# robflynnyh/long-context-asr

Hardware: AMD Instinct MI355X
Metric: spectrogram-frames/sec (6L/768D, seq=16384) (higher is better)
Workload: dtype bf16; 1 GPU; 6L/768D/6H SConformerXL, seq=16384, rotary theta=1.5M, fwd+CTC+bwd+clip+MADGRAD; per_gpu_batch=128, global_batch=128, seq_len=16384, parallelism=dp1

## Files before the change

long-context-asr_amd/csrc/gemm256.hip:

```cpp
#ifdef SCONF_GEMM_STAMP
#define SCONF_STAMPS
#endif
#include "gemm_tile.h"
#include <algorithm>
#include <stdio.h>

namespace {
using namespace gemm_tile;

constexpr int TM = 256, TK = 64;
constexpr int HT = 128 * 64 * 2;
constexpr int BUF = 4 * HT;
constexpr int GM2 = 4;

__device__ __forceinline__ int swz_a(int row) { return (row >> 1) & 7; }
__device__ __forceinline__ int swz_b(int row) { return ((row >> 1) & 1) | (((row >> 3) & 3) << 1); }
__device__ __forceinline__ int swz_b1n(int row) { return ((row >> 1) & 1) | (((row >> 2) & 3) << 1); }

template <bool KS, bool BOP, int JH> struct DmaOffs {
    unsigned off[2][2];
    __device__ __forceinline__ void set(long ld, int tid, bool rot = false) {
        constexpr int WC = 32 + 16 * JH;
#pragma unroll
        for (int h = 0; h < 2; ++h)
#pragma unroll
            for (int i = 0; i < 2; ++i) {
                const int c = tid + 512 * i;
                if (!KS) {
                    const int row = c >> 3, pos = c & 7;
                    int kc, mrow;
                    if (!BOP)              { kc = pos ^ swz_a(row); mrow = 128 * h + row; }
                    else if (h == 0)       { kc = pos ^ swz_b(row); mrow = rot ? 128 * (row >> 6) + 32 * ((row >> 5) & 1) + (row & 31) : WC * (row >> 5) + (row & 31); }
                    else if (JH == 2)      { kc = pos ^ swz_b(row); mrow = rot ? 128 * (row >> 6) + 32 * ((row >> 5) & 1) + 64 + (row & 31) : WC * (row >> 5) + 32 + (row & 31); }
                    else                   { kc = pos ^ swz_b1n(row & 63); mrow = WC * ((row & 63) >> 4) + 32 + (row & 15); }
                    off[h][i] = (unsigned)(((long)mrow * ld + kc * 8) * 2);
                } else {
                    const int kr = c >> 4, pos = c & 15, rc = pos ^ swz_strided(kr);
                    off[h][i] = (unsigned)(((long)kr * ld + 128 * h + rc * 8) * 2);
                }
            }
    }
};
template <int NP>
__device__ __forceinline__ void dma_half(const char* base, const unsigned (&off)[2], char* dst, int tid) {
#pragma unroll
    for (int i = 0; i < NP; ++i)
        __builtin_amdgcn_global_load_lds((gptr)(base + off[i]), (lptr)(dst + ((tid & ~63) + 512 * i) * 16), 16, 0, 0);
}

__device__ __forceinline__ bf16x4 lds_read_tr(const char* p) {
    bf16x4 v;
    asm volatile("ds_read_b64_tr_b16 %0, %1" : "=v"(v) : "v"(lds_addr(p)));
    return v;
}
template <int OFF> __device__ __forceinline__ bf16x4 lds_read_tr_off(unsigned a) {
    bf16x4 v;
    asm volatile("ds_read_b64_tr_b16 %0, %1 offset:%2" : "=v"(v) : "v"(a), "n"(OFF));
    return v;
}
__device__ __forceinline__ void frag_pair_ks(const char* s, int col, int lane, bf16x8& f0, bf16x8& f1) {
    const int a = lane & 15, q = a >> 2, g = lane >> 4;
    const int chunk = col >> 3, sub = (col & 4) * 2, k0 = 8 * g + q;
    const unsigned base = lds_addr(s + k0 * 256 + ((chunk ^ swz_strided(k0)) << 4) + sub);
    const bf16x4 l0 = lds_read_tr_off<0>(base), h0 = lds_read_tr_off<1024>(base);
    const bf16x4 l1 = lds_read_tr_off<8192>(base), h1 = lds_read_tr_off<9216>(base);
    f0 = __builtin_shufflevector(l0, h0, 0, 1, 2, 3, 4, 5, 6, 7);
    f1 = __builtin_shufflevector(l1, h1, 0, 1, 2, 3, 4, 5, 6, 7);
}
template <bool KS> __device__ __forceinline__ bf16x8 frag_a(const char* s, int wr, int i, int kk, int lane) {
    if (!KS) {
        const int r = 64 * wr + 16 * i + (lane & 15), c = kk * 4 + (lane >> 4);
        return *reinterpret_cast<const bf16x8*>(s + r * 128 + ((c ^ swz_a(r)) << 4));
    } else {
        const int a = lane & 15, q = a >> 2, pp = a & 3, g = lane >> 4;
        const int col = 64 * wr + 16 * i + 4 * pp, chunk = col >> 3, sub = (col & 4) * 2;
        const int k0 = kk * 32 + 8 * g + q, k1 = k0 + 4;
        bf16x4 lo = lds_read_tr(s + k0 * 256 + ((chunk ^ swz_strided(k0)) << 4) + sub);
        bf16x4 hi = lds_read_tr(s + k1 * 256 + ((chunk ^ swz_strided(k1)) << 4) + sub);
        return __builtin_shufflevector(lo, hi, 0, 1, 2, 3, 4, 5, 6, 7);
    }
}
template <bool KS, bool NARROW> __device__ __forceinline__ bf16x8 frag_b(const char* s, int wc, int j, int kk, int lane) {
    if (!KS) {
        const int a = lane & 15, c = kk * 4 + (lane >> 4);
        if (!NARROW) {
            const int r = 32 * wc + 8 * (a >> 2) + 4 * j + (a & 3);
            return *reinterpret_cast<const bf16x8*>(s + r * 128 + ((c ^ swz_b(r)) << 4));
        } else {
            const int r = 16 * wc + 4 * (a >> 2) + (a & 3);
            return *reinterpret_cast<const bf16x8*>(s + r * 128 + ((c ^ swz_b1n(r)) << 4));
        }
    } else {
        const int a = lane & 15, q = a >> 2, pp = a & 3, g = lane >> 4;
        const int col = 32 * wc + 16 * j + 4 * pp, chunk = col >> 3, sub = (col & 4) * 2;
        const int k0 = kk * 32 + 8 * g + q, k1 = k0 + 4;
        bf16x4 lo = lds_read_tr(s + k0 * 256 + ((chunk ^ swz_strided(k0)) << 4) + sub);
        bf16x4 hi = lds_read_tr(s + k1 * 256 + ((chunk ^ swz_strided(k1)) << 4) + sub);
        return __builtin_shufflevector(lo, hi, 0, 1, 2, 3, 4, 5, 6, 7);
    }
}

struct Item { int m0, n0, kbeg, nkt, split; };
struct Sched { int total, ntiles, tiles_m, tiles_n, tn, gm; };
__device__ __forceinline__ Item item_coords(const GemmParams& p, const Sched& sc, int v) {
    const int qx = sc.total >> 3, rx = sc.total & 7, xcd = v & 7;
    const int lid = (xcd < rx ? xcd * (qx + 1) : rx * (qx + 1) + (xcd - rx) * qx) + (v >> 3);
    const int split = lid / sc.ntiles, t = lid - split * sc.ntiles;
    const int per_group = sc.gm * sc.tiles_n;
    const int g = t / per_group, r = t - g * per_group;
    const int first_m = g * sc.gm, gm = min(sc.gm, sc.tiles_m - first_m);
    Item w;
    w.m0 = (first_m + r % gm) * TM; w.n0 = (r / gm) * sc.tn;
    w.split = split;
    w.kbeg = split * p.k_per_split;
    w.nkt = (min(p.K, w.kbeg + p.k_per_split) - w.kbeg) / TK;
    return w;
}
struct Cursor {
    int v, kt, par; bool valid; Item it;
    __device__ __forceinline__ void advance(const GemmParams& p, const Sched& sc) {
        par ^= 1;
        if (++kt < it.nkt) return;
        kt = 0; v += gridDim.x;
        if (v < sc.total) it = item_coords(p, sc, v); else valid = false;
    }
};

template <int W> struct RawBf;
template <> struct RawBf<8> { typedef bf16x8 type; };
template <> struct RawBf<4> { typedef bf16x4 type; };
template <int ACT, bool RES, bool KS, int JH, int FL = -1, bool ROT = false, int DEEP = 0>
__device__ __forceinline__ void epilogue256(const GemmParams& p, const f32x4 (&acc)[2][4][2 + JH], const Item& it, int wr, int wc, int lane) {
    constexpr int WC = 32 + 16 * JH, WH = 4 * JH;
    constexpr bool AUX = ACT == SCONF_ACT_DGELU || ACT == SCONF_ACT_DSILU || ACT == SCONF_ACT_MULAUX || ACT == SCONF_ACT_SMAXBWD;
    constexpr bool SMB = ACT == SCONF_ACT_SMAXBWD;
    const int g = lane >> 4, mbase = it.m0 + 64 * wr + (lane & 15);
    if constexpr (ROT) {
        static_assert(JH == 2 && !RES && !AUX && ACT == SCONF_ACT_NONE && FL >= 0 && !(FL & 2), "rotary epilogue: 256-wide tile, plain bf16 output");
        const int d0 = 32 * (wc & 1) + 8 * g;
        const int nlo = it.n0 + 128 * (wc >> 1) + d0, nhi = nlo + 64;
        float blo[8], bhi[8];
#pragma unroll
        for (int e = 0; e < 8; ++e) { blo[e] = 0.f; bhi[e] = 0.f; }
        if (FL & 1) { loadv<8>(p.bias + nlo, blo); loadv<8>(p.bias + nhi, bhi); }
        const bool rot = it.n0 < p.rot_cols;
        const long crow0 = (long)mbase * p.ldc;
        float cs[2][8], sn[2][8];
        auto fetch = [&](int rb, int slot) {
            const int pos = (mbase + 128 * (rb >> 2) + 16 * (rb & 3)) % p.rot_n;
            loadv<8>(p.rot_cos + (long)pos * 64 + d0, cs[slot]); loadv<8>(p.rot_sin + (long)pos * 64 + d0, sn[slot]);
        };
        if (rot) fetch(0, 0);
#pragma unroll
        for (int rb = 0; rb < 8; ++rb) {
            if (rot && rb + 1 < 8) fetch(rb + 1, (rb + 1) & 1);
            const int h = rb >> 2, i = rb & 3, sl = rb & 1;
            float lo[8], hi[8];
#pragma unroll
            for (int e = 0; e < 8; ++e) { lo[e] = acc[h][i][e >> 2][e & 3] + blo[e]; hi[e] = acc[h][i][2 + (e >> 2)][e & 3] + bhi[e]; }
            if (rot) {
#pragma unroll
                for (int e = 0; e < 8; ++e) {
                    const float a = lo[e], b = hi[e];
                    lo[e] = a * cs[sl][e] - b * sn[sl][e]; hi[e] = b * cs[sl][e] + a * sn[sl][e];
                }
            }
            const long crow = crow0 + (long)(128 * h + 16 * i) * p.ldc;
            storev<8>(reinterpret_cast<bf16*>(p.C) + crow + nlo, lo); storev<8>(reinterpret_cast<bf16*>(p.C) + crow + nhi, hi);
        }
        return;
    }
    if constexpr (!KS) {
        const int nlo = it.n0 + WC * wc + 8 * g, nhi = it.n0 + WC * wc + 32 + WH * g;
        float blo[8], bhi[WH];
#pragma unroll
        for (int e = 0; e < 8; ++e) blo[e] = 0.f;
#pragma unroll
        for (int e = 0; e < WH; ++e) bhi[e] = 0.f;
        if (FL >= 0 ? (FL & 1) != 0 : p.bias != nullptr) { loadv<8>(p.bias + nlo, blo); loadv<WH>(p.bias + nhi, bhi); }
        const long crow0 = (long)mbase * p.ldc, prow0 = (long)mbase * p.ldpre;
        if constexpr (FL >= 0 && (RES || ACT == SCONF_ACT_MULAUX || SMB)) {
            constexpr int NB = 8;
            constexpr int NS = DEEP ? (RES ? (JH == 2 ? 4 : 5) : 8) : (RES ? (JH == 2 ? 2 : 3) : 5);
            constexpr bool FIXED = RES || DEEP;
            float rl[NS][8], rh[NS][WH];
            typename RawBf<8>::type xl[NS];
            typename RawBf<WH>::type xh[NS];
            float rowv[NS], cslo[8], cshi[WH];
            if constexpr (SMB) {
#pragma unroll
                for (int e = 0; e < 8; ++e) cslo[e] = 0.f;
#pragma unroll
                for (int e = 0; e < WH; ++e) cshi[e] = 0.f;
            }
            auto fetch = [&](int rb, int slot) {
                const int row = mbase + 128 * (rb >> 2) + 16 * (rb & 3);
                if constexpr (SMB) rowv[slot] = p.rowv[row];
                if constexpr (RES) { const float* q = p.resid + (long)row * p.ldr; loadv<8>(q + nlo, rl[slot]); loadv<WH>(q + nhi, rh[slot]); }
                if constexpr (AUX) {
                    const bf16* q = p.aux + (long)row * p.ldaux;
                    xl[slot] = *reinterpret_cast<const typename RawBf<8>::type*>(q + nlo);
                    xh[slot] = *reinterpret_cast<const typename RawBf<WH>::type*>(q + nhi);
                }
            };
#pragma unroll
            for (int nb = 0; nb < (FIXED ? NS - 1 : 1); ++nb) fetch(nb, nb);
#pragma unroll
            for (int rb = 0; rb < NB; ++rb) {
                {
                    const int lo_b = FIXED ? rb + NS - 1 : (rb == 0 ? 1 : 2 * rb), hi_b = FIXED ? rb + NS - 1 : 2 * rb + 1;
#pragma unroll
                    for (int nb = lo_b; nb <= hi_b; ++nb) if (nb < NB) fetch(nb, nb % NS);
                }
                const int h = rb >> 2, i = rb & 3, sl = rb % NS;
                float vlo[8], vhi[WH], alo[8], ahi[WH], zlo[8], zhi[WH];
#pragma unroll
                for (int e = 0; e < 8; ++e) { vlo[e] = acc[h][i][e >> 2][e & 3]; alo[e] = AUX ? (float)xl[sl][e] : 0.f; zlo[e] = RES ? rl[sl][e] : (SMB ? rowv[sl] : 0.f); }
#pragma unroll
                for (int e = 0; e < WH; ++e) { vhi[e] = acc[h][i][2 + (e >> 2)][e & 3]; ahi[e] = AUX ? (float)xh[sl][e] : 0.f; zhi[e] = RES ? rh[sl][e] : (SMB ? rowv[sl] : 0.f); }
                const long crow = crow0 + (long)(128 * h + 16 * i) * p.ldc, prow = prow0 + (long)(128 * h + 16 * i) * p.ldpre;
                epi_math_store_at<8, ACT, FL>(p, vlo, blo, alo, zlo, crow + nlo, prow + nlo, it.split);
                epi_math_store_at<WH, ACT, FL>(p, vhi, bhi, ahi, zhi, crow + nhi, prow + nhi, it.split);
                if constexpr (SMB) {
#pragma unroll
                    for (int e = 0; e < 8; ++e) cslo[e] += vlo[e];
#pragma unroll
                    for (int e = 0; e < WH; ++e) cshi[e] += vhi[e];
                }
            }
            if constexpr (SMB) {
                auto row_sum = [](float v) {
                    v += __int_as_float(__builtin_amdgcn_update_dpp(0, __float_as_int(v), 0xB1, 0xF, 0xF, true));
                    v += __int_as_float(__builtin_amdgcn_update_dpp(0, __float_as_int(v), 0x4E, 0xF, 0xF, true));
                    v += __int_as_float(__builtin_amdgcn_update_dpp(0, __float_as_int(v), 0x141, 0xF, 0xF, true));
                    v += __int_as_float(__builtin_amdgcn_update_dpp(0, __float_as_int(v), 0x140, 0xF, 0xF, true));
                    return v;
                };
#pragma unroll
                for (int e = 0; e < 8; ++e) cslo[e] = row_sum(cslo[e]);
#pragma unroll
                for (int e = 0; e < WH; ++e) cshi[e] = row_sum(cshi[e]);
                if ((lane & 15) == 0) {
                    float* q = p.colslab + (long)(2 * (it.m0 / TM) + wr) * p.N;
                    storev<8>(q + nlo, cslo); storev<WH>(q + nhi, cshi);
                }
            }
            return;
        }
#pragma unroll
        for (int h = 0; h < 2; ++h) {
            typename RawBf<8>::type axlo[4];
            typename RawBf<WH>::type axhi[4];
            if constexpr (AUX) {
#pragma unroll
                for (int i = 0; i < 4; ++i) {
                    const bf16* q = p.aux + (long)(mbase + 128 * h + 16 * i) * p.ldaux;
                    axlo[i] = *reinterpret_cast<const typename RawBf<8>::type*>(q + nlo);
                    axhi[i] = *reinterpret_cast<const typename RawBf<WH>::type*>(q + nhi);
                }
            }
#pragma unroll
            for (int i2 = 0; i2 < 4; i2 += 2) {
                float rlo[2][8], rhi[2][WH];
#pragma unroll
                for (int ii = 0; ii < 2; ++ii) {
#pragma unroll
                    for (int e = 0; e < 8; ++e) rlo[ii][e] = 0.f;
#pragma unroll
                    for (int e = 0; e < WH; ++e) rhi[ii][e] = 0.f;
                    if constexpr (RES) {
                        const float* q = p.resid + (long)(mbase + 128 * h + 16 * (i2 + ii)) * p.ldr;
                        loadv<8>(q + nlo, rlo[ii]); loadv<WH>(q + nhi, rhi[ii]);
                    }
                }
#pragma unroll
                for (int ii = 0; ii < 2; ++ii) {
                    const int i = i2 + ii;
                    float vlo[8], vhi[WH], alo[8], ahi[WH];
#pragma unroll
                    for (int e = 0; e < 8; ++e) { vlo[e] = acc[h][i][e >> 2][e & 3]; alo[e] = AUX ? (float)axlo[i][e] : 0.f; }
#pragma unroll
                    for (int e = 0; e < WH; ++e) { vhi[e] = acc[h][i][2 + (e >> 2)][e & 3]; ahi[e] = AUX ? (float)axhi[i][e] : 0.f; }
                    const long crow = crow0 + (long)(128 * h + 16 * i) * p.ldc, prow = prow0 + (long)(128 * h + 16 * i) * p.ldpre;
                    epi_math_store_at<8, ACT, FL>(p, vlo, blo, alo, rlo[ii], crow + nlo, prow + nlo, it.split);
                    epi_math_store_at<WH, ACT, FL>(p, vhi, bhi, ahi, rhi[ii], crow + nhi, prow + nhi, it.split);
                }
            }
        }
    } else {
        const int nb = it.n0 + 32 * wc + 4 * g;
        const int ncol[4] = {nb, nb + 16, nb + 128, nb + 144};
        float zero[4] = {0.f, 0.f, 0.f, 0.f}, bs[4][4];
#pragma unroll
        for (int j = 0; j < 4; ++j) {
#pragma unroll
            for (int e = 0; e < 4; ++e) bs[j][e] = 0.f;
            if (p.bias) loadv<4>(p.bias + ncol[j], bs[j]);
        }
#pragma unroll
        for (int h = 0; h < 2; ++h)
#pragma unroll
            for (int i = 0; i < 4; ++i)
#pragma unroll
                for (int j = 0; j < 4; ++j) {
                    float v[4] = {acc[h][i][j][0], acc[h][i][j][1], acc[h][i][j][2], acc[h][i][j][3]};
                    epi_math_store<4, ACT>(p, v, bs[j], zero, zero, mbase + 128 * h + 16 * i, ncol[j], it.split);
                }
    }
}

__host__ __device__ __forceinline__ int epilogue_kind(const GemmParams& p) {
    if (p.rot_cos) return p.bias ? 8 : 7;
    const bool b = p.bias != nullptr, unit = p.alpha == 1.f;
    if (p.act == SCONF_ACT_GELU_DSAVE) return (!b && !p.out_f32 && !p.resid && unit) ? 4 : 6;
    if (p.act == SCONF_ACT_MULAUX) return (!b && !p.out_f32 && !p.resid && !p.pre) ? 5 : 6;
    if (p.act == SCONF_ACT_SMAXBWD) return 10;
    if (p.act == SCONF_ACT_NONE && p.pre && p.out_f32 && p.resid && b) return 9;
    if (p.act != SCONF_ACT_NONE || p.pre) return 6;
    if (!p.out_f32 && !p.resid) return unit ? (b ? 1 : 0) : 6;
    if (p.out_f32 && p.resid) return b ? 3 : 2;
    if (p.out_f32 && unit) return b ? 12 : 11;
    return 6;
}
#define EPILOGUE_NT(JH_)                                                                                              \
    switch (ekind) {                                                                                                  \
        case 0: epilogue256<SCONF_ACT_NONE, false, false, JH_, 4>(p, acc, cit, wr, wc, lane); break;                  \
        case 1: epilogue256<SCONF_ACT_NONE, false, false, JH_, 5>(p, acc, cit, wr, wc, lane); break;                  \
        case 2: epilogue256<SCONF_ACT_NONE, true, false, JH_, 2>(p, acc, cit, wr, wc, lane); break;                   \
        case 3: epilogue256<SCONF_ACT_NONE, true, false, JH_, 3>(p, acc, cit, wr, wc, lane); break;                   \
        case 4: epilogue256<SCONF_ACT_GELU_DSAVE, false, false, JH_, 4>(p, acc, cit, wr, wc, lane); break;            \
        case 5: epilogue256<SCONF_ACT_MULAUX, false, false, JH_, 0>(p, acc, cit, wr, wc, lane); break;                \
        case 7: if constexpr (JH_ == 2) epilogue256<SCONF_ACT_NONE, false, false, JH_, 0, true>(p, acc, cit, wr, wc, lane); break;  \
        case 8: if constexpr (JH_ == 2) epilogue256<SCONF_ACT_NONE, false, false, JH_, 1, true>(p, acc, cit, wr, wc, lane); break;  \
        default:                                                                                                      \
            if (p.act == SCONF_ACT_GELU_DSAVE)  epilogue256<SCONF_ACT_GELU_DSAVE, false, false, JH_>(p, acc, cit, wr, wc, lane); \
            else if (p.act == SCONF_ACT_MULAUX) epilogue256<SCONF_ACT_MULAUX, false, false, JH_>(p, acc, cit, wr, wc, lane);     \
            else if (p.resid)                   epilogue256<SCONF_ACT_NONE, true, false, JH_>(p, acc, cit, wr, wc, lane);        \
            else                                epilogue256<SCONF_ACT_NONE, false, false, JH_>(p, acc, cit, wr, wc, lane);       \
    }

#ifndef DEEPV
#define DEEPV 1
#endif
#define EPILOGUE_ONE(EK_, JH_)                                                                                        \
    do {                                                                                                              \
        if constexpr (EK_ == 0) epilogue256<SCONF_ACT_NONE, false, false, JH_, 4>(p, acc, cit, wr, wc, lane);         \
        else if constexpr (EK_ == 1) epilogue256<SCONF_ACT_NONE, false, false, JH_, 5>(p, acc, cit, wr, wc, lane);    \
        else if constexpr (EK_ == 2) epilogue256<SCONF_ACT_NONE, true, false, JH_, 2, false, DEEPV>(p, acc, cit, wr, wc, lane);     \
        else if constexpr (EK_ == 3) epilogue256<SCONF_ACT_NONE, true, false, JH_, 3, false, DEEPV>(p, acc, cit, wr, wc, lane);     \
        else if constexpr (EK_ == 4) epilogue256<SCONF_ACT_GELU_DSAVE, false, false, JH_, 4>(p, acc, cit, wr, wc, lane); \
        else if constexpr (EK_ == 5) epilogue256<SCONF_ACT_MULAUX, false, false, JH_, 0, false, DEEPV>(p, acc, cit, wr, wc, lane);  \
        else if constexpr (EK_ == 7) epilogue256<SCONF_ACT_NONE, false, false, JH_, 0, true>(p, acc, cit, wr, wc, lane); \
        else if constexpr (EK_ == 8) epilogue256<SCONF_ACT_NONE, false, false, JH_, 1, true>(p, acc, cit, wr, wc, lane); \
        else if constexpr (EK_ == 9) epilogue256<SCONF_ACT_NONE, true, false, JH_, 11, false, DEEPV>(p, acc, cit, wr, wc, lane);    \
        else if constexpr (EK_ == 11) epilogue256<SCONF_ACT_NONE, false, false, JH_, 6>(p, acc, cit, wr, wc, lane);   \
        else if constexpr (EK_ == 12) epilogue256<SCONF_ACT_NONE, false, false, JH_, 7>(p, acc, cit, wr, wc, lane);   \
        else epilogue256<SCONF_ACT_SMAXBWD, false, false, JH_, 4, false, DEEPV>(p, acc, cit, wr, wc, lane);                         \
    } while (0)

#ifdef SCONF_GEMM_STAMP
__device__ unsigned long long g_gemm_stamps[256 * 8 * 8];
#define STAMP_OUT do { if ((threadIdx.x & 63) == 0 && blockIdx.x < 256) for (int i_ = 0; i_ < 8; ++i_) g_gemm_stamps[((long)blockIdx.x * 8 + (threadIdx.x >> 6)) * 8 + i_] = st_acc_[i_]; } while (0)
#else
#define STAMP_OUT
#endif
template <int JH> __device__ __forceinline__ void wait_window(bool streaming) {
    if (!streaming) wait_vm<0>();
    else if (JH == 2) wait_vm<8>();
    else wait_vm<7>();
}

template <bool KS, int EK = -1>
__global__ __launch_bounds__(512) void gemm256_kernel(const GemmParams p) {
    constexpr int JH = 2, TN = 256;
    extern __shared__ __attribute__((aligned(16))) char smem[];
    const int tid = threadIdx.x, lane = tid & 63;
    const int wave = __builtin_amdgcn_readfirstlane(tid >> 6);
    const int wr = wave >> 2, wc = wave & 3;
    Sched sc;
    sc.tn = TN; sc.tiles_n = p.N / TN; sc.tiles_m = p.M / TM; sc.ntiles = sc.tiles_m * sc.tiles_n; sc.total = sc.ntiles * p.splits; sc.gm = sc.tiles_n >= 8 ? 2 * GM2 : GM2;
    if ((int)blockIdx.x >= sc.total) return;

    const int ekind = __builtin_amdgcn_readfirstlane(epilogue_kind(p));
    DmaOffs<KS, false, JH> oa; DmaOffs<KS, true, JH> ob;
    oa.set(p.lda, tid); ob.set(p.ldb, tid, !KS && p.rot_cos != nullptr);
    auto issue_a = [&](const Cursor& c, int h) {
        if (!c.valid) return;
        const long k0 = c.it.kbeg + c.kt * TK;
        const char* base = reinterpret_cast<const char*>(p.A) + (KS ? k0 * p.lda + c.it.m0 : (long)c.it.m0 * p.lda + k0) * 2;
        dma_half<2>(base, oa.off[h], smem + c.par * BUF + h * HT, tid);
    };
    auto issue_b = [&](const Cursor& c, int h) {
        if (!c.valid) return;
        const long k0 = c.it.kbeg + c.kt * TK;
        const char* base = reinterpret_cast<const char*>(p.B) + (KS ? k0 * p.ldb + c.it.n0 : (long)c.it.n0 * p.ldb + k0) * 2;
        if (h == 0) dma_half<2>(base, ob.off[0], smem + c.par * BUF + 2 * HT, tid);
        else        dma_half<JH>(base, ob.off[1], smem + c.par * BUF + 3 * HT, tid);
    };

    f32x4 acc[2][4][2 + JH];
#pragma unroll
    for (int h = 0; h < 2; ++h)
#pragma unroll
        for (int i = 0; i < 4; ++i)
#pragma unroll
            for (int j = 0; j < 2 + JH; ++j) acc[h][i][j] = f32x4{0.f, 0.f, 0.f, 0.f};

    Cursor pc;
    pc.v = blockIdx.x; pc.kt = 0; pc.par = 0; pc.valid = true; pc.it = item_coords(p, sc, pc.v);
    int cv = pc.v; Item cit = pc.it;
    issue_a(pc, 0); issue_b(pc, 0); issue_b(pc, 1); issue_a(pc, 1);
    pc.advance(p, sc);
    issue_a(pc, 0); issue_b(pc, 0);
    if (pc.valid) wait_window<JH>(true);
    else wait_vm<4>();
    __builtin_amdgcn_s_barrier();

    int cur = 0;
    bf16x8 fa[4][2], blo[2][2], bhi[JH][2];
    STAMP_DECL(8)
    while (true) {
        if (wr) __builtin_amdgcn_s_barrier();
        for (int kt = 0; kt < cit.nkt; ++kt) {
            const char* buf = smem + cur * BUF;
            const bool last = kt == cit.nkt - 1;
#pragma unroll
            for (int j = 0; j < 2; ++j) {
                if constexpr (KS) frag_pair_ks(buf + 2 * HT, 32 * wc + 16 * j + 4 * (lane & 3), lane, blo[j][0], blo[j][1]);
                else {
#pragma unroll
                    for (int kk = 0; kk < 2; ++kk) blo[j][kk] = frag_b<KS, false>(buf + 2 * HT, wc, j, kk, lane);
                }
            }
#pragma unroll
            for (int i = 0; i < 4; ++i) {
                if constexpr (KS) frag_pair_ks(buf, 64 * wr + 16 * i + 4 * (lane & 3), lane, fa[i][0], fa[i][1]);
                else {
#pragma unroll
                    for (int kk = 0; kk < 2; ++kk) fa[i][kk] = frag_a<KS>(buf, wr, i, kk, lane);
                }
            }
            STAMP(6);
            issue_b(pc, 1);
            STAMP(7);
            wait_window<JH>(pc.valid);
            STAMP(0);
            __builtin_amdgcn_s_barrier();
            STAMP(1);
            if constexpr (KS) {
                wait_lgkm0();
#pragma unroll
                for (int kk = 0; kk < 2; ++kk) {
#pragma unroll
                    for (int j = 0; j < 2; ++j) tie(blo[j][kk]);
#pragma unroll
                    for (int i = 0; i < 4; ++i) tie(fa[i][kk]);
                }
            }
            __builtin_amdgcn_s_setprio(1);
#pragma unroll
            for (int kk = 0; kk < 2; ++kk)
#pragma unroll
                for (int i = 0; i < 4; ++i)
#pragma unroll
                    for (int j = 0; j < 2; ++j)
                        acc[0][i][j] = __builtin_amdgcn_mfma_f32_16x16x32_bf16(blo[j][kk], fa[i][kk], acc[0][i][j], 0, 0, 0);
            __builtin_amdgcn_s_setprio(0);
            STAMP(2);
            __builtin_amdgcn_s_barrier();
            STAMP(3);
#pragma unroll
            for (int j = 0; j < JH; ++j) {
                if constexpr (KS) frag_pair_ks(buf + 3 * HT, 32 * wc + 16 * j + 4 * (lane & 3), lane, bhi[j][0], bhi[j][1]);
                else {
#pragma unroll
                    for (int kk = 0; kk < 2; ++kk) bhi[j][kk] = frag_b<KS, false>(buf + 3 * HT, wc, j, kk, lane);
                }
            }
            STAMP(6);
            issue_a(pc, 1);
            STAMP(7);
            wait_window<JH>(pc.valid);
            STAMP(0);
            __builtin_amdgcn_s_barrier();
            STAMP(1);
            if constexpr (KS) {
                wait_lgkm0();
#pragma unroll
                for (int kk = 0; kk < 2; ++kk)
#pragma unroll
                    for (int j = 0; j < JH; ++j) tie(bhi[j][kk]);
            }
            __builtin_amdgcn_s_setprio(1);
#pragma unroll
            for (int kk = 0; kk < 2; ++kk)
#pragma unroll
                for (int i = 0; i < 4; ++i)
#pragma unroll
                    for (int j = 0; j < JH; ++j)
                        acc[0][i][2 + j] = __builtin_amdgcn_mfma_f32_16x16x32_bf16(bhi[j][kk], fa[i][kk], acc[0][i][2 + j], 0, 0, 0);
            __builtin_amdgcn_s_setprio(0);
            STAMP(2);
            __builtin_amdgcn_s_barrier();
            STAMP(3);
#pragma unroll
            for (int i = 0; i < 4; ++i) {
                if constexpr (KS) frag_pair_ks(buf + HT, 64 * wr + 16 * i + 4 * (lane & 3), lane, fa[i][0], fa[i][1]);
                else {
#pragma unroll
                    for (int kk = 0; kk < 2; ++kk) fa[i][kk] = frag_a<KS>(buf + HT, wr, i, kk, lane);
                }
            }
            pc.advance(p, sc);
            STAMP(6);
            issue_a(pc, 0);
            STAMP(7);
            wait_window<JH>(pc.valid);
            STAMP(0);
            __builtin_amdgcn_s_barrier();
            STAMP(1);
            if constexpr (KS) {
                wait_lgkm0();
#pragma unroll
                for (int kk = 0; kk < 2; ++kk)
#pragma unroll
                    for (int i = 0; i < 4; ++i) tie(fa[i][kk]);
            }
            __builtin_amdgcn_s_setprio(1);
#pragma unroll
            for (int kk = 0; kk < 2; ++kk)
#pragma unroll
                for (int i = 0; i < 4; ++i)
#pragma unroll
                    for (int j = 0; j < JH; ++j)
                        acc[1][i][2 + j] = __builtin_amdgcn_mfma_f32_16x16x32_bf16(bhi[j][kk], fa[i][kk], acc[1][i][2 + j], 0, 0, 0);
            __builtin_amdgcn_s_setprio(0);
            STAMP(2);
            __builtin_amdgcn_s_barrier();
            STAMP(3);
            STAMP(6);
            issue_b(pc, 0);
            STAMP(7);
            wait_window<JH>(pc.valid);
            STAMP(0);
            __builtin_amdgcn_s_barrier();
            STAMP(1);
            __builtin_amdgcn_s_setprio(1);
#pragma unroll
            for (int kk = 0; kk < 2; ++kk)
#pragma unroll
                for (int i = 0; i < 4; ++i)
#pragma unroll
                    for (int j = 0; j < 2; ++j)
                        acc[1][i][j] = __builtin_amdgcn_mfma_f32_16x16x32_bf16(blo[j][kk], fa[i][kk], acc[1][i][j], 0, 0, 0);
            __builtin_amdgcn_s_setprio(0);
            STAMP(2);
            if (!(wr && last)) __builtin_amdgcn_s_barrier();
            STAMP(3);
            cur ^= 1;
        }
        if constexpr (KS) epilogue256<SCONF_ACT_NONE, false, true, JH>(p, acc, cit, wr, wc, lane);
        else if constexpr (EK >= 0) EPILOGUE_ONE(EK, JH);
        else EPILOGUE_NT(JH);
#pragma unroll
        for (int h = 0; h < 2; ++h)
#pragma unroll
            for (int i = 0; i < 4; ++i)
#pragma unroll
                for (int j = 0; j < 2 + JH; ++j) acc[h][i][j] = f32x4{0.f, 0.f, 0.f, 0.f};
        STAMP(4);
        __builtin_amdgcn_s_barrier();
        STAMP(5);
        cv += gridDim.x;
        if (cv >= sc.total) break;
        cit = item_coords(p, sc, cv);
    }
    wait_vm<0>();
    STAMP_OUT;
}

template <int EK = -1>
__global__ __launch_bounds__(512) void gemm192_kernel(const GemmParams p) {
    constexpr int JH = 1, WC = 48, TN = 192;
    extern __shared__ __attribute__((aligned(16))) char smem[];
    const int tid = threadIdx.x, lane = tid & 63;
    const int wave = __builtin_amdgcn_readfirstlane(tid >> 6);
    const int wr = wave >> 2, wc = wave & 3;
    Sched sc;
    sc.tn = TN; sc.tiles_n = p.N / TN; sc.tiles_m = p.M / TM; sc.ntiles = sc.tiles_m * sc.tiles_n; sc.total = sc.ntiles * p.splits; sc.gm = sc.tiles_n >= 8 ? 2 * GM2 : GM2;
    if ((int)blockIdx.x >= sc.total) return;

    const int ekind = __builtin_amdgcn_readfirstlane(epilogue_kind(p));
    DmaOffs<false, false, JH> oa; DmaOffs<false, true, JH> ob;
    oa.set(p.lda, tid); ob.set(p.ldb, tid);
    auto issue_a = [&](const Cursor& c, int h) {
        if (!c.valid) return;
        const long k0 = c.it.kbeg + c.kt * TK;
        dma_half<2>(reinterpret_cast<const char*>(p.A) + ((long)c.it.m0 * p.lda + k0) * 2, oa.off[h], smem + c.par * BUF + h * HT, tid);
    };
    auto issue_b = [&](const Cursor& c, int h) {
        if (!c.valid) return;
        const long k0 = c.it.kbeg + c.kt * TK;
        const char* base = reinterpret_cast<const char*>(p.B) + ((long)c.it.n0 * p.ldb + k0) * 2;
        if (h == 0) dma_half<2>(base, ob.off[0], smem + c.par * BUF + 2 * HT, tid);
        else        dma_half<1>(base, ob.off[1], smem + c.par * BUF + 3 * HT, tid);
    };

    f32x4 acc[2][4][3];
#pragma unroll
    for (int h = 0; h < 2; ++h)
#pragma unroll
        for (int i = 0; i < 4; ++i)
#pragma unroll
            for (int j = 0; j < 3; ++j) acc[h][i][j] = f32x4{0.f, 0.f, 0.f, 0.f};

    Cursor pc;
    pc.v = blockIdx.x; pc.kt = 0; pc.par = 0; pc.valid = true; pc.it = item_coords(p, sc, pc.v);
    int cv = pc.v; Item cit = pc.it;
    issue_a(pc, 0); issue_b(pc, 0); issue_a(pc, 1); issue_b(pc, 1);
    pc.advance(p, sc);
    issue_a(pc, 0); issue_b(pc, 0);
    if (pc.valid) wait_vm<7>(); else wait_vm<3>();
    __builtin_amdgcn_s_barrier();

    int cur = 0;
    bf16x8 flo[4][2], fhi[4][2], blo[2][2], bhi[2];
    while (true) {
        if (wr) __builtin_amdgcn_s_barrier();
        for (int kt = 0; kt < cit.nkt; ++kt) {
            const char* buf = smem + cur * BUF;
            const bool last = kt == cit.nkt - 1;
#pragma unroll
            for (int j = 0; j < 2; ++j)
#pragma unroll
                for (int kk = 0; kk < 2; ++kk) blo[j][kk] = frag_b<false, false>(buf + 2 * HT, wc, j, kk, lane);
#pragma unroll
            for (int i = 0; i < 4; ++i)
#pragma unroll
                for (int kk = 0; kk < 2; ++kk) flo[i][kk] = frag_a<false>(buf, wr, i, kk, lane);
            issue_a(pc, 1); issue_b(pc, 1);
            wait_window<JH>(pc.valid);
            __builtin_amdgcn_s_barrier();
            __builtin_amdgcn_s_setprio(1);
#pragma unroll
            for (int kk = 0; kk < 2; ++kk)
#pragma unroll
                for (int i = 0; i < 4; ++i)
#pragma unroll
                    for (int j = 0; j < 2; ++j)
                        acc[0][i][j] = __builtin_amdgcn_mfma_f32_16x16x32_bf16(blo[j][kk], flo[i][kk], acc[0][i][j], 0, 0, 0);
            __builtin_amdgcn_s_setprio(0);
            __builtin_amdgcn_s_barrier();
#pragma unroll
            for (int kk = 0; kk < 2; ++kk) bhi[kk] = frag_b<false, true>(buf + 3 * HT, wc, 0, kk, lane);
#pragma unroll
            for (int i = 0; i < 4; ++i)
#pragma unroll
                for (int kk = 0; kk < 2; ++kk) fhi[i][kk] = frag_a<false>(buf + HT, wr, i, kk, lane);
            __builtin_amdgcn_s_barrier();
            __builtin_amdgcn_s_setprio(1);
#pragma unroll
            for (int kk = 0; kk < 2; ++kk)
#pragma unroll
                for (int i = 0; i < 4; ++i) {
                    acc[0][i][2] = __builtin_amdgcn_mfma_f32_16x16x32_bf16(bhi[kk], flo[i][kk], acc[0][i][2], 0, 0, 0);
                    acc[1][i][2] = __builtin_amdgcn_mfma_f32_16x16x32_bf16(bhi[kk], fhi[i][kk], acc[1][i][2], 0, 0, 0);
                }
            __builtin_amdgcn_s_setprio(0);
            __builtin_amdgcn_s_barrier();
            pc.advance(p, sc);
            issue_a(pc, 0); issue_b(pc, 0);
            wait_window<JH>(pc.valid);
            __builtin_amdgcn_s_barrier();
            __builtin_amdgcn_s_setprio(1);
#pragma unroll
            for (int kk = 0; kk < 2; ++kk)
#pragma unroll
                for (int i = 0; i < 4; ++i)
#pragma unroll
                    for (int j = 0; j < 2; ++j)
                        acc[1][i][j] = __builtin_amdgcn_mfma_f32_16x16x32_bf16(blo[j][kk], fhi[i][kk], acc[1][i][j], 0, 0, 0);
            __builtin_amdgcn_s_setprio(0);
            if (!(wr && last)) __builtin_amdgcn_s_barrier();
            cur ^= 1;
        }
        if constexpr (EK >= 0) EPILOGUE_ONE(EK, JH);
        else EPILOGUE_NT(JH);
#pragma unroll
        for (int h = 0; h < 2; ++h)
#pragma unroll
            for (int i = 0; i < 4; ++i)
#pragma unroll
                for (int j = 0; j < 3; ++j) acc[h][i][j] = f32x4{0.f, 0.f, 0.f, 0.f};
        __builtin_amdgcn_s_barrier();
        cv += gridDim.x;
        if (cv >= sc.total) break;
        cit = item_coords(p, sc, cv);
    }
    wait_vm<0>();
}

}

static int pick_width(const GemmParams& p, int layout, int cus) {
    if (p.M % TM || p.K % TK || p.k_per_split % TK) return 0;
    if (p.rot_cos) return (layout == 0 && p.N % 256 == 0) ? 256 : 0;
    long best = 0; int bw = 0;
    for (int w : {256, 192}) {
        if (p.N % w || (w == 192 && layout != 0)) continue;
        const long items = (long)(p.M / TM) * (p.N / w) * p.splits;
        const long cost = ((items + cus - 1) / cus) * w * (w == 192 ? 9 : 8);
        if (!bw || cost < best) { best = cost; bw = w; }
    }
    return bw;
}

bool sconf_gemm256_eligible(const GemmParams& p, int layout) {
    if (layout != 0 && layout != 2) return false;
    const bool ks = layout == 2;
    if (ks ? (p.act != SCONF_ACT_NONE || p.resid || p.pre)
           : !(p.act == SCONF_ACT_NONE || ((p.act == SCONF_ACT_GELU_DSAVE || p.act == SCONF_ACT_MULAUX) && !p.resid) ||
               (p.act == SCONF_ACT_SMAXBWD && !p.resid && !p.bias && !p.out_f32 && !p.pre && p.splits == 1))) return false;
    if ((ks ? 64 : 256) * p.lda * 2 >= (1L << 32) || (ks ? 64 : 256) * p.ldb * 2 >= (1L << 32)) return false;
    const int cus = num_cus();
    const int w = pick_width(p, layout, cus);
    if (!w || (p.act == SCONF_ACT_SMAXBWD && w != 256)) return false;
    return (long)(p.M / TM) * (p.N / w) * p.splits * 4 >= 3L * cus;
}

int sconf_gemm256_width(const GemmParams& p, int layout) { return pick_width(p, layout, num_cus()); }

int sconf_gemm256_launch(const GemmParams& p, int layout, hipStream_t stream) {
    static bool attr_set = false;
    const size_t shmem = 2 * BUF;
    lds_limit_once(attr_set, {(const void*)gemm256_kernel<false>, (const void*)gemm256_kernel<true>,
                             (const void*)gemm256_kernel<false, 0>, (const void*)gemm256_kernel<false, 1>, (const void*)gemm256_kernel<false, 2>,
                             (const void*)gemm256_kernel<false, 3>, (const void*)gemm256_kernel<false, 4>, (const void*)gemm256_kernel<false, 5>,
                             (const void*)gemm256_kernel<false, 7>, (const void*)gemm256_kernel<false, 8>, (const void*)gemm256_kernel<false, 9>,
                             (const void*)gemm256_kernel<false, 10>, (const void*)gemm256_kernel<false, 11>, (const void*)gemm256_kernel<false, 12>,
                             (const void*)gemm192_kernel<11>, (const void*)gemm192_kernel<12>, (const void*)gemm192_kernel<-1>, (const void*)gemm192_kernel<0>,
                             (const void*)gemm192_kernel<1>, (const void*)gemm192_kernel<2>, (const void*)gemm192_kernel<3>, (const void*)gemm192_kernel<4>,
                             (const void*)gemm192_kernel<5>, (const void*)gemm192_kernel<9>}, shmem);
    const int cus = num_cus();
    const int w = pick_width(p, layout, cus);
    const int total = (p.M / TM) * (p.N / w) * p.splits;
    dim3 grid(std::min(total, cus)), block(512);
    const int ek = layout == 2 ? -1 : epilogue_kind(p);
#define L256(EK_) hipLaunchKernelGGL((gemm256_kernel<false, EK_>), grid, block, shmem, stream, p)
#define L192(EK_) hipLaunchKernelGGL(gemm192_kernel<EK_>, grid, block, shmem, stream, p)
    if (layout == 2)   hipLaunchKernelGGL((gemm256_kernel<true>), grid, block, shmem, stream, p);
    else if (w == 256) {
        switch (ek) {
            case 0: L256(0); break; case 1: L256(1); break; case 2: L256(2); break; case 3: L256(3); break; case 4: L256(4); break;
            case 5: L256(5); break; case 7: L256(7); break; case 8: L256(8); break; case 9: L256(9); break; case 10: L256(10); break;
            case 11: L256(11); break; case 12: L256(12); break;
            default: L256(-1);
        }
    } else {
        switch (ek) {
            case 0: L192(0); break; case 1: L192(1); break; case 2: L192(2); break; case 3: L192(3); break; case 4: L192(4); break;
            case 5: L192(5); break; case 9: L192(9); break; case 11: L192(11); break; case 12: L192(12); break;
            default: L192(-1);
        }
    }
#undef L256
#undef L192
    SCONF_LAUNCH_OK("sconf_gemm_bf16 (256-row tile)");
#ifdef SCONF_GEMM_STAMP
    if (getenv("SCONF_GEMM_STAMP_PRINT") && (layout == 2 || w == 256)) {
        (void)hipStreamSynchronize(stream);
        static unsigned long long hb[256 * 8 * 8];
        (void)hipMemcpyFromSymbol(hb, HIP_SYMBOL(g_gemm_stamps), sizeof(hb));
        const int nwg = std::min(total, 256);
        const double ktiles = (double)total / nwg * (p.k_per_split / TK);
        static const char* nm[8] = {"vmcnt wait", "barrier 1", "MFMA cluster", "barrier 2", "epilogue", "re-align", "frag reads", "DMA issue"};
        for (int g = 0; g < 2; ++g) {
            double sums[8] = {}, tot = 0;
            for (int wg = 0; wg < nwg; ++wg) for (int wv = 4 * g; wv < 4 * g + 4; ++wv) for (int i = 0; i < 8; ++i) sums[i] += (double)hb[(wg * 8 + wv) * 8 + i];
            for (int i = 0; i < 8; ++i) tot += sums[i];
            fprintf(stderr, "[gemm256 %s M=%d N=%d K=%d stamps] wave row %d: cycles per K-tile %.0f:", layout == 2 ? "TN" : "NT", p.M, p.N, p.K, g, tot / (nwg * 4.0 * ktiles));
            for (int i = 0; i < 8; ++i) fprintf(stderr, "  %s %.0f (%.1f%%)", nm[i], sums[i] / (nwg * 4.0 * ktiles), 100.0 * sums[i] / tot);
            fprintf(stderr, "\n");
        }
    }
#endif
    return 0;
}
```

Baseline: 7.024 million spectrogram-frames/sec.

## Overlap GEMM epilogue stores with next tile's K-loop via quadrant retirement

Adds a ROLL variant of the 256x256 persistent GEMM kernel for three common epilogue kinds (plain bf16, GELU-save, f32 out). On the last K-tile, each accumulator quadrant is written out and zeroed as soon as its MFMAs finish, interleaved with the next tile's prologue DMA. The vmcnt wait windows are widened to account for the extra outstanding stores. The goal is to hide epilogue store latency and remove the full post-tile barrier stall. The cost is more complex vmcnt accounting, which risks over-waiting, and extra register and code pressure. It is on by default, with an env var to disable it.

```diff
diff --git a/long-context-asr_amd/csrc/gemm256.hip b/long-context-asr_amd/csrc/gemm256.hip
--- a/long-context-asr_amd/csrc/gemm256.hip
+++ b/long-context-asr_amd/csrc/gemm256.hip
@@ -306,6 +306,28 @@
                     float v[4] = {acc[h][i][j][0], acc[h][i][j][1], acc[h][i][j][2], acc[h][i][j][3]};
                     epi_math_store<4, ACT>(p, v, bs[j], zero, zero, mbase + 128 * h + 16 * i, ncol[j], it.split);
                 }
+    }
+}
+
+template <int EK> struct RollKind { static constexpr bool on = false; static constexpr int act = SCONF_ACT_NONE, fl = 4, ops = 0; };
+template <> struct RollKind<0>  { static constexpr bool on = true; static constexpr int act = SCONF_ACT_NONE, fl = 4, ops = 4; };
+template <> struct RollKind<4>  { static constexpr bool on = true; static constexpr int act = SCONF_ACT_GELU_DSAVE, fl = 4, ops = 8; };
+template <> struct RollKind<11> { static constexpr bool on = true; static constexpr int act = SCONF_ACT_NONE, fl = 6, ops = 8; };
+template <int EK, int Q>
+__device__ __forceinline__ void retire_quadrant(const GemmParams& p, f32x4 (&acc)[2][4][4], const Item& it, int wr, int wc, int lane) {
+    constexpr int h = Q >> 1, jb = (Q == 1 || Q == 2) ? 2 : 0;
+    lane = opaque(lane);
+    const int g = lane >> 4, mbase = it.m0 + 64 * wr + (lane & 15) + 128 * h;
+    const int n = it.n0 + 64 * wc + 8 * g + (jb ? 32 : 0);
+    const float zero[8] = {0.f, 0.f, 0.f, 0.f, 0.f, 0.f, 0.f, 0.f};
+#pragma unroll
+    for (int i = 0; i < 4; ++i) {
+        float v[8];
+#pragma unroll
+        for (int e = 0; e < 8; ++e) v[e] = acc[h][i][jb + (e >> 2)][e & 3];
+        const long row = mbase + 16 * i;
+        epi_math_store_at<8, RollKind<EK>::act, RollKind<EK>::fl>(p, v, zero, zero, zero, row * p.ldc + n, row * p.ldpre + n, it.split);
+        acc[h][i][jb] = f32x4{0.f, 0.f, 0.f, 0.f}; acc[h][i][jb + 1] = f32x4{0.f, 0.f, 0.f, 0.f};
     }
 }
 
@@ -370,7 +392,17 @@
     else wait_vm<7>();
 }
 
-template <bool KS, int EK = -1>
+__device__ __forceinline__ int uniform_opaque(int v) { v = __builtin_amdgcn_readfirstlane(v); asm volatile("" : "+s"(v)); return v; }
+template <int E, int KL, int KF, int KFL> __device__ __forceinline__ void wait_window_roll(bool streaming, bool last, bool fresh) {
+    static_assert(8 + 4 * E < 64, "vmcnt is a 6-bit field");
+    if (!streaming) wait_vm<0>();
+    else if (fresh) { if (last) wait_vm<8 + KFL * E>(); else wait_vm<8 + KF * E>(); }
+    else if (last) wait_vm<8 + KL * E>();
+    else wait_vm<8>();
+}
+#define ROLL_RETIRE(Q) do { if constexpr (ROLL) { if (last) { retire_quadrant<EK, Q>(p, acc, cit, wr, wc, lane); STAMP(4); } } } while (0)
+
+template <bool KS, int EK = -1, bool ROLL = false>
 __global__ __launch_bounds__(512) void gemm256_kernel(const GemmParams p) {
     constexpr int JH = 2, TN = 256;
     extern __shared__ __attribute__((aligned(16))) char smem[];
@@ -418,12 +450,14 @@
 
     int cur = 0;
     bf16x8 fa[4][2], blo[2][2], bhi[JH][2];
+    bool rolled = false;
     STAMP_DECL(8)
     while (true) {
         if (wr) __builtin_amdgcn_s_barrier();
         for (int kt = 0; kt < cit.nkt; ++kt) {
             const char* buf = smem + cur * BUF;
-            const bool last = kt == cit.nkt - 1;
+            const bool last = ROLL ? uniform_opaque(kt == cit.nkt - 1) != 0 : kt == cit.nkt - 1;
+            const bool fresh = ROLL && uniform_opaque(rolled && kt == 0) != 0;
 #pragma unroll
             for (int j = 0; j < 2; ++j) {
                 if constexpr (KS) frag_pair_ks(buf + 2 * HT, 32 * wc + 16 * j + 4 * (lane & 3), lane, blo[j][0], blo[j][1]);
@@ -443,7 +477,8 @@
             STAMP(6);
             issue_b(pc, 1);
             STAMP(7);
-            wait_window<JH>(pc.valid);
+            if constexpr (ROLL) wait_window_roll<RollKind<EK>::ops, 0, 4, 4>(pc.valid, last, fresh);
+            else wait_window<JH>(pc.valid);
             STAMP(0);
             __builtin_amdgcn_s_barrier();
             STAMP(1);
@@ -480,7 +515,9 @@
             STAMP(6);
             issue_a(pc, 1);
             STAMP(7);
-            wait_window<JH>(pc.valid);
+            ROLL_RETIRE(0);
+            if constexpr (ROLL) wait_window_roll<RollKind<EK>::ops, 1, 3, 4>(pc.valid, last, fresh);
+            else wait_window<JH>(pc.valid);
             STAMP(0);
             __builtin_amdgcn_s_barrier();
             STAMP(1);
@@ -515,7 +552,9 @@
             STAMP(6);
             issue_a(pc, 0);
             STAMP(7);
-            wait_window<JH>(pc.valid);
+            ROLL_RETIRE(1);
+            if constexpr (ROLL) wait_window_roll<RollKind<EK>::ops, 2, 2, 4>(pc.valid, last, fresh);
+            else wait_window<JH>(pc.valid);
             STAMP(0);
             __builtin_amdgcn_s_barrier();
             STAMP(1);
@@ -541,7 +580,9 @@
             STAMP(6);
             issue_b(pc, 0);
             STAMP(7);
-            wait_window<JH>(pc.valid);
+            ROLL_RETIRE(2);
+            if constexpr (ROLL) wait_window_roll<RollKind<EK>::ops, 3, 0, 3>(pc.valid, last, fresh);
+            else wait_window<JH>(pc.valid);
             STAMP(0);
             __builtin_amdgcn_s_barrier();
             STAMP(1);
@@ -559,18 +600,28 @@
             STAMP(3);
             cur ^= 1;
         }
-        if constexpr (KS) epilogue256<SCONF_ACT_NONE, false, true, JH>(p, acc, cit, wr, wc, lane);
-        else if constexpr (EK >= 0) EPILOGUE_ONE(EK, JH);
-        else EPILOGUE_NT(JH);
-#pragma unroll
-        for (int h = 0; h < 2; ++h)
-#pragma unroll
-            for (int i = 0; i < 4; ++i)
-#pragma unroll
-                for (int j = 0; j < 2 + JH; ++j) acc[h][i][j] = f32x4{0.f, 0.f, 0.f, 0.f};
-        STAMP(4);
-        __builtin_amdgcn_s_barrier();
-        STAMP(5);
+        if constexpr (ROLL) {
+            if (!wr) retire_quadrant<EK, 3>(p, acc, cit, wr, wc, lane);
+            STAMP(4);
+            __builtin_amdgcn_s_barrier();
+            STAMP(5);
+            if (wr) retire_quadrant<EK, 3>(p, acc, cit, wr, wc, lane);
+            STAMP(4);
+            rolled = true;
+        } else {
+            if constexpr (KS) epilogue256<SCONF_ACT_NONE, false, true, JH>(p, acc, cit, wr, wc, lane);
+            else if constexpr (EK >= 0) EPILOGUE_ONE(EK, JH);
+            else EPILOGUE_NT(JH);
+#pragma unroll
+            for (int h = 0; h < 2; ++h)
+#pragma unroll
+                for (int i = 0; i < 4; ++i)
+#pragma unroll
+                    for (int j = 0; j < 2 + JH; ++j) acc[h][i][j] = f32x4{0.f, 0.f, 0.f, 0.f};
+            STAMP(4);
+            __builtin_amdgcn_s_barrier();
+            STAMP(5);
+        }
         cv += gridDim.x;
         if (cv >= sc.total) break;
         cit = item_coords(p, sc, cv);
@@ -740,15 +791,23 @@
                              (const void*)gemm256_kernel<false, 10>, (const void*)gemm256_kernel<false, 11>, (const void*)gemm256_kernel<false, 12>,
                              (const void*)gemm192_kernel<11>, (const void*)gemm192_kernel<12>, (const void*)gemm192_kernel<-1>, (const void*)gemm192_kernel<0>,
                              (const void*)gemm192_kernel<1>, (const void*)gemm192_kernel<2>, (const void*)gemm192_kernel<3>, (const void*)gemm192_kernel<4>,
-                             (const void*)gemm192_kernel<5>, (const void*)gemm192_kernel<9>}, shmem);
+                             (const void*)gemm192_kernel<5>, (const void*)gemm192_kernel<9>,
+                             (const void*)gemm256_kernel<false, 0, true>, (const void*)gemm256_kernel<false, 4, true>,
+                             (const void*)gemm256_kernel<false, 11, true>}, shmem);
     const int cus = num_cus();
     const int w = pick_width(p, layout, cus);
     const int total = (p.M / TM) * (p.N / w) * p.splits;
     dim3 grid(std::min(total, cus)), block(512);
     const int ek = layout == 2 ? -1 : epilogue_kind(p);
+    static const bool roll_on = [] { const char* e = getenv("SCONF_GEMM_ROLL"); return !(e && e[0] == '0'); }();
+    const bool roll = roll_on && layout == 0 && w == 256 && p.splits == 1;
 #define L256(EK_) hipLaunchKernelGGL((gemm256_kernel<false, EK_>), grid, block, shmem, stream, p)
+#define R256(EK_) hipLaunchKernelGGL((gemm256_kernel<false, EK_, true>), grid, block, shmem, stream, p)
 #define L192(EK_) hipLaunchKernelGGL(gemm192_kernel<EK_>, grid, block, shmem, stream, p)
     if (layout == 2)   hipLaunchKernelGGL((gemm256_kernel<true>), grid, block, shmem, stream, p);
+    else if (roll && ek == 0) R256(0);
+    else if (roll && ek == 4) R256(4);
+    else if (roll && ek == 11) R256(11);
     else if (w == 256) {
         switch (ek) {
             case 0: L256(0); break; case 1: L256(1); break; case 2: L256(2); break; case 3: L256(3); break; case 4: L256(4); break;
@@ -764,6 +823,7 @@
         }
     }
 #undef L256
+#undef R256
 #undef L192
     SCONF_LAUNCH_OK("sconf_gemm_bf16 (256-row tile)");
 #ifdef SCONF_GEMM_STAMP
```

Measured after the change: 6.758 million spectrogram-frames/sec. -3.8%, worse.
